# xxlong0/NeuralUDF

Hardware: AMD Instinct MI355X
Metric: ray-samples/sec (train step) (higher is better)
Workload: dtype f32 emulated on the 16-bit matrix pipe, f32 accumulate, f32 state / epilogues / optimizer.  Forward-order sweeps (UDF value, input gradient, colour / NeRF forward): f16x2 (x = hi + 2^-11 lo in fp16, 3 fp16 MFMA products, correction terms in their own accumulator).  Backward sweeps (tangent, adjoint

## Files before the change

### include/nudf.h

```cpp
#ifndef NUDF_H
#define NUDF_H
#include <stdint.h>

#ifdef __cplusplus
extern "C" {
#endif

#define NUDF_ABI_VERSION 111
int nudf_version(void);
#define NUDF_ABI_STRUCTS(X) \
  X(NudfGemmNN) X(NudfGemmTN) X(NudfGemmTNProblem) X(NudfGemmTNGroup) X(NudfComposite) X(NudfCompositeGrad) \
  X(NudfUpsample) X(NudfPixelBlend) X(NudfPixelComposite) X(NudfPatchBlend) X(NudfPatchWarp) X(NudfBlendLoss) \
  X(NudfAdamTensor) X(NudfAdamGroup) X(NudfAdam) X(NudfChainStep) X(NudfChain) X(NudfPackFrag) X(NudfPackLayer) \
  X(NudfPackMulti) X(NudfUnpackLayer) X(NudfUnpackMulti) X(NudfRayBatch) X(NudfMeshUDF) X(NudfMeshUDFSparse) \
  X(NudfIsoSurface) X(NudfIsoSurfaceSparse) X(NudfPointCloud) X(NudfMeshTopo) X(NudfMeshOrient) X(NudfMeshRaster)
int nudf_abi_struct(int i, const char** name);
const char* nudf_last_error(void);

enum {
  NUDF_STATUS_NONFINITE_RENDER = 1,
  NUDF_STATUS_NONFINITE_SAMPLES = 2,
  NUDF_STATUS_NONFINITE_LOSS = 4
};
int nudf_set_status_flag(int32_t* device_word);
// ... 354 lines not shown
  const float* X3;
  int32_t ldx3;
} NudfChainStep;
#define NUDF_CH_BLK_X1 1
#define NUDF_CH_BLK_X2 2
#define NUDF_CH_BLK_C1 4
#define NUDF_CH_BLK_C2 8
#define NUDF_CH_BLK_PE 16
#define NUDF_CH_STATE16 32
#define NUDF_CH_P4_X1 64
#define NUDF_CH_P4_C1 128
typedef struct NudfChain {
  int32_t P, n_steps;
  int32_t init;
  int32_t k0;
  int32_t x_div;
  int32_t tile_rows;
  int32_t lda0, ldg0;
  int32_t pe_L, pe_jvp;
  int32_t init_state16;
  float pe_in_scale;
  float seed_scale, seed_xscale;
  const float* A0;
  float* G0;
  const float* x;
  const float* v;
  const float* seed_sign;
  const float* seed_wrow;
  unsigned long long* dbg;
  float* absmax_out;
  const float* tile_amax_in;
  float* tile_amax_out;
  int32_t tile_scale;
  int32_t reserved0;
  NudfChainStep step[NUDF_CH_MAX_STEPS];
} NudfChain;
#define NUDF_CH_TILE_TQ 66
#define NUDF_CH_TILE_ROWS 128
#if defined(__cplusplus)
static_assert(sizeof(NudfChain) <= 4096, "NudfChain travels by value: the kernel-argument segment holds 4 KB");
#endif
int nudf_mlp_chain(const NudfChain* args, void* stream);
int nudf_mlp_chain_plan(const NudfChain* args, char* name, int capacity, int32_t* out);
int nudf_set_chain_t16(int on);
int nudf_pack_frag(const float* B, int ldb, int K, int N, float* out, void* stream);

#define NUDF_PACK_MAX_LAYERS 16
#define NUDF_PACK_MAX_FRAGS 4
typedef struct NudfPackFrag {
  float* dst;
  int32_t transpose;
  int32_t o0, i0;
  int32_t K, N;
  int32_t dtype;
} NudfPackFrag;
typedef struct NudfPackLayer {
  const float* v; const float* g;
  const int32_t* perm;
  float* W; float* Wt;
  float* inv_norm;
  int32_t out, in, ldw, ldwt;
  int32_t nfrag, row_start;
  NudfPackFrag frag[NUDF_PACK_MAX_FRAGS];
} NudfPackLayer;
typedef struct NudfPackMulti {
  int32_t n_layers, total_rows;
  NudfPackLayer layer[NUDF_PACK_MAX_LAYERS];
// ... 508 lines not shown
```

### neuraludf_amd/_lib.py

```python
from __future__ import annotations

import ctypes as C
import os

import torch

_HERE = os.path.dirname(os.path.abspath(__file__))
LIB_PATH = os.environ.get("NUDF_LIB") or os.path.join(_HERE, "libnudf.so")
ABI_VERSION = 111

c_fp = C.c_void_p
i32 = C.c_int32
f32 = C.c_float


class NudfError(RuntimeError):
    pass


class GemmNN(C.Structure):
    _fields_ = [("A", c_fp), ("lda", i32), ("B", c_fp), ("ldb", i32), ("bias", c_fp),
                ("C1", c_fp), ("ldc1", i32), ("C2", c_fp), ("ldc2", i32), ("C3", c_fp), ("ldc3", i32),
                ("X1", c_fp), ("ldx1", i32), ("X2", c_fp), ("ldx2", i32),
                ("M", i32), ("N", i32), ("K", i32), ("epi", i32), ("iparam", i32), ("scale", f32), ("xscale", f32)]
# ... 101 lines not shown

class AdamGroup(C.Structure):
    _fields_ = [("one_minus_beta1", f32), ("beta2", f32), ("one_minus_beta2", f32), ("eps", f32)]


class Adam(C.Structure):
    _fields_ = [("n_tensors", i32), ("pad_", i32), ("t", AdamTensor * ADAM_MAX_TENSORS),
                ("block_start", i32 * (ADAM_MAX_TENSORS + 1)), ("pad2_", i32), ("group", AdamGroup * ADAM_MAX_GROUPS),
                ("dyn", c_fp)]


CH_MAX_STEPS = 20
CH_STATE16 = 32
CH_P4_X1, CH_P4_C1 = 64, 128
CH = dict(NONE=0, SOFTPLUS=1, MULSP=2, TANGENT=3, BWD=4, UDFHEAD=5, RELU=6, SIGMOIDN=7, MULMASK=8, ADDMASK=9, RELUADD=10,
          SEED=11)
CH_INIT = dict(LOAD=0, POSENC=1, SEED=2)


class ChainStep(C.Structure):
    _fields_ = [("Bp", c_fp), ("bias", c_fp), ("X1", c_fp), ("X2", c_fp), ("C1", c_fp), ("C2", c_fp),
                ("r1_row", c_fp), ("r1_col", c_fp), ("K", i32), ("N", i32), ("epi", i32), ("iparam", i32),
                ("ldx1", i32), ("ldx2", i32), ("ldc1", i32), ("ldc2", i32), ("ldr1", i32), ("prec", i32), ("act_write", i32),
                ("act_col0", i32), ("pe_tail_col", i32), ("ld_pe", i32), ("pe_dst", c_fp), ("pe_tail_scale", f32),
                ("scale", f32), ("xscale", f32), ("layout", i32), ("row_w", c_fp), ("row_sums", c_fp), ("X3", c_fp),
                ("ldx3", i32)]


class Chain(C.Structure):
    _fields_ = [("P", i32), ("n_steps", i32), ("init", i32), ("k0", i32), ("x_div", i32), ("tile_rows", i32), ("lda0", i32),
                ("ldg0", i32), ("pe_L", i32), ("pe_jvp", i32), ("init_state16", i32), ("pe_in_scale", f32), ("seed_scale", f32),
                ("seed_xscale", f32), ("A0", c_fp), ("G0", c_fp), ("x", c_fp), ("v", c_fp), ("seed_sign", c_fp),
                ("seed_wrow", c_fp), ("dbg", c_fp), ("absmax_out", c_fp), ("tile_amax_in", c_fp),
                ("tile_amax_out", c_fp), ("tile_scale", C.c_int32), ("reserved0", C.c_int32), ("step", ChainStep * CH_MAX_STEPS)]


PACK_MAX_LAYERS = 16
PACK_MAX_FRAGS = 4


class PackFrag(C.Structure):
    _fields_ = [("dst", c_fp), ("transpose", i32), ("o0", i32), ("i0", i32), ("K", i32), ("N", i32), ("dtype", i32)]


class PackLayer(C.Structure):
    _fields_ = [("v", c_fp), ("g", c_fp), ("perm", c_fp), ("W", c_fp), ("Wt", c_fp), ("inv_norm", c_fp),
                ("out", i32), ("in_", i32), ("ldw", i32), ("ldwt", i32), ("nfrag", i32), ("row_start", i32),
                ("frag", PackFrag * PACK_MAX_FRAGS)]


class PackMulti(C.Structure):
    _fields_ = [("n_layers", i32), ("total_rows", i32), ("layer", PackLayer * PACK_MAX_LAYERS)]


class UnpackLayer(C.Structure):
    _fields_ = [("dW", c_fp), ("v", c_fp), ("g", c_fp), ("inv_norm", c_fp), ("perm", c_fp), ("dv", c_fp),
                ("dg", c_fp), ("db_in", c_fp), ("db_out", c_fp), ("out", i32), ("in_", i32), ("ldw", i32), ("row_start", i32)]


class UnpackMulti(C.Structure):
    _fields_ = [("n_layers", i32), ("total_rows", i32), ("layer", UnpackLayer * PACK_MAX_LAYERS)]


class MeshUDF(C.Structure):
    _fields_ = [("U", c_fp), ("G", c_fp), ("axes", c_fp), ("cell_case", c_fp), ("cell_ntri", c_fp), ("edge_flag", c_fp),
                ("cells", c_fp), ("face_off", c_fp), ("edge_scan", c_fp), ("faces", c_fp), ("edges", c_fp), ("verts", c_fp),
                ("n_cells", C.c_int64), ("n_edges", C.c_int64), ("n_faces", C.c_int64), ("N", i32), ("mean_thr", f32),
# ... 332 lines not shown
```

### neuraludf_amd/csrc/mlp_chain.hip

```cpp
#include "nudf_common.h"
#include "../../include/nudf.h"

#include "mlp_chain_shared.h"
#include <stdlib.h>
#include <type_traits>

template <int TM>
struct ChainSmem {
  float act[TM * CH_LD];
  float xs[TM * 3];
  float vs[TM * 3];
  float red[8];
};
#define CH_SGN_COL 288
static_assert(CH_SGN_COL < CH_LD, "the head multiplier lives in the tile's row padding");

template <int TM>
struct ChainSmem16 {
  unsigned short act[TM * CH_LD16];
  float xs[TM * 3];
  float vs[TM * 3];
  float red[8];
};

template <int TM, class SM>
__device__ __forceinline__ void ch_write_pe(SM& sm, const NudfChain& p, int m0, int col0, float scale,
                                            float* gdst, int ldg, int gcol0, int zero_to, bool dst16 = false, int tfmt = 0,
                                            float gscale = 1.0f) {
  ch_write_pe_rows<CH_THREADS>(reinterpret_cast<float*>(sm.act), sm.xs, sm.vs, TM, threadIdx.x, p, m0, col0, scale, gdst, ldg,
                               gcol0, zero_to, dst16, false, tfmt, gscale);
}


struct ChPrefetch {
  const float* X1;
  int ldx1;
  unsigned vo[2][2];
};

template <int NRT, int NCT, bool PF>
__device__ __forceinline__ void ch_mma(const float* __restrict__ arow, const f32x4* __restrict__ bptr, size_t bstride,
                                       int G, f32x16 (&acc)[2][2], const ChPrefetch& pf, float (&px1)[2][2][16]) {
  f32x4 a0[NRT], a1[NRT], b0[NCT], b1[NCT];
#pragma unroll
  for (int i = 0; i < NRT; ++i) a0[i] = *reinterpret_cast<const f32x4*>(arow + i * 32 * CH_LD);
#pragma unroll
  for (int j = 0; j < NCT; ++j) b0[j] = bptr[j * 64];
#pragma unroll 1
  for (int g = 0; g < G - 2; g += 2) {
    {
      const f32x4* bq = bptr + (size_t)(g + 1) * bstride;
#pragma unroll
      for (int j = 0; j < NCT; ++j) b1[j] = bq[j * 64];
#pragma unroll
      for (int i = 0; i < NRT; ++i) a1[i] = *reinterpret_cast<const f32x4*>(arow + i * 32 * CH_LD + (g + 1) * 8);
    }
    __builtin_amdgcn_sched_barrier(0);
#pragma unroll
    for (int jj = 0; jj < 4; ++jj)
#pragma unroll
      for (int i = 0; i < NRT; ++i)
#pragma unroll
        for (int j = 0; j < NCT; ++j) acc[i][j] = ch_mfma(a0[i][jj], b0[j][jj], acc[i][j]);
// ... 1016 lines not shown
    for (int e = tid; e < TM * k4; e += CH_THREADS) {
      const int r = e / k4, c4 = e - r * k4;
      int gr = m0 + r;
      if (gr > p.P - 1) gr = p.P - 1;
      const f32x4 val = *reinterpret_cast<const f32x4*>(p.A0 + (size_t)gr * p.lda0 + c4 * 4);
      if constexpr (X3) amax = fmaxf(amax, fmaxf(fmaxf(fabsf(val[0]), fabsf(val[1])), fmaxf(fabsf(val[2]), fabsf(val[3]))));
      if constexpr (T16) {
        uint2 w;
        if (tile_bf) {
          w.x = (unsigned)ch_f2bf(val[0]) | ((unsigned)ch_f2bf(val[1]) << 16);
          w.y = (unsigned)ch_f2bf(val[2]) | ((unsigned)ch_f2bf(val[3]) << 16);
        } else {
          w.x = ch_f2h2(val[0], val[1]);
          w.y = ch_f2h2(val[2], val[3]);
        }
        *reinterpret_cast<uint2*>(sm.act + r * CH_LD16 + c4 * 4) = w;
      } else {
        *reinterpret_cast<f32x4*>(act_f + r * CH_LD + c4 * 4) = val;
      }
    }
    if constexpr (X3) {
      if (tscale) {
        set_sigma(wg_max(fmaxf(amax, other_seeds())));
        for (int e = tid; e < TM * k4; e += CH_THREADS) {
          const int r = e / k4, c4 = e - r * k4;
          f32x4* q = reinterpret_cast<f32x4*>(act_f + r * CH_LD + c4 * 4);
          f32x4 val = *q;
          val[0] *= tsig; val[1] *= tsig; val[2] *= tsig; val[3] *= tsig;
          *q = val;
        }
      }
    }
  } else if (p.init == NUDF_CH_INIT_POSENC) {
    ch_write_pe<TM>(sm, p, m0, 0, 1.0f, p.G0, p.ldg0, 0, p.k0, false, tfmt, tinv);
  } else if (p.init == NUDF_CH_INIT_SEED) {
    const int C = p.k0;
    if ((p.init_state16 & 3) == 3 && p.G0) {
      const uint2* A4 = reinterpret_cast<const uint2*>(p.A0);
      uint2* G4 = reinterpret_cast<uint2*>(p.G0);
      for (int e = tid; e < (TM / 4) * C; e += CH_THREADS) {
        const int q = e / C, c = e - q * C;
        const unsigned gq = (unsigned)(m0 >> 2) + (unsigned)q;
        float hst[4], val[4];
        ch_p4_widen(A4[(size_t)gq * p.lda0 + c], hst);
#pragma unroll
        for (int k = 0; k < 4; ++k) {
          int gr = m0 + 4 * q + k;
          if (gr > p.P - 1) gr = p.P - 1;
          float sd, om;
          ch_sp_derivs(hst[k], p.seed_xscale, sd, om);
          val[k] = p.seed_sign[gr] * p.seed_wrow[c] * p.seed_scale * sd;
          const int r = 4 * q + k;
          if constexpr (T16) sm.act[r * CH_LD16 + c] = tile_bf ? ch_f2bf(val[k]) : ch_f2h(val[k]);
          else act_f[r * CH_LD + c] = val[k];
        }
        uint2 w;
        w.x = (unsigned)ch_f2bf(val[0]) | ((unsigned)ch_f2bf(val[1]) << 16);
        w.y = (unsigned)ch_f2bf(val[2]) | ((unsigned)ch_f2bf(val[3]) << 16);
        G4[(size_t)gq * p.ldg0 + c] = w;
      }
    } else
    for (int e = tid; e < TM * C; e += CH_THREADS) {
      const int r = e / C, c = e - r * C;
      int gr = m0 + r;
      const bool live = gr < p.P;
      if (!live) gr = p.P - 1;
      float s, om;
      const float hst = (p.init_state16 & 1) ? ch_bf2f(reinterpret_cast<const unsigned short*>(p.A0)[ch_p4_off(gr, c, p.lda0)])
                                             : p.A0[(size_t)gr * p.lda0 + c];
      ch_sp_derivs(hst, p.seed_xscale, s, om);
      const float val = p.seed_sign[gr] * p.seed_wrow[c] * p.seed_scale * s;
      if constexpr (T16) sm.act[r * CH_LD16 + c] = tile_bf ? ch_f2bf(val) : ch_f2h(val);
      else act_f[r * CH_LD + c] = val;
      if (p.G0 && live) {
        if (p.init_state16 & 2) reinterpret_cast<unsigned short*>(p.G0)[ch_p4_off(gr, c, p.ldg0)] = ch_f2bf(val);
        else p.G0[(size_t)gr * p.ldg0 + c] = val;
      }
    }
  }
  __syncthreads();

  const unsigned slot = __builtin_amdgcn_s_getreg((3 << 11) | (0 << 6) | 4);
  if (gridDim.x > 256) {
    constexpr unsigned STAGGER16 = 0u, STAGGER32 = 2u;
    const unsigned k = (ANY16 || X3) ? (slot & 1u) * STAGGER16 : ((TM == 64) ? (slot & 1u) * STAGGER32 : slot % 3u);
    for (unsigned d = 0; d < k; ++d) __builtin_amdgcn_s_sleep(127);
  }

  unsigned long long* dbg = p.dbg ? p.dbg + ((size_t)blockIdx.x * 4 + wave) * 64 : nullptr;
  if (dbg && lane == 0) {
    dbg[0] = __builtin_amdgcn_s_getreg((31 << 11) | (0 << 6) | 4);
    dbg[1] = __builtin_amdgcn_s_memtime();
    dbg[62] = wall_clock64();
  }

  for (int si = 0; si < p.n_steps; ++si) {
    const NudfChainStep& st = p.step[si];
    if ((si + slot) & 1u) __builtin_amdgcn_s_setprio(1); else __builtin_amdgcn_s_setprio(0);
    if constexpr (X3) {
      if (st.epi == NUDF_CH_SEED) {
        int t = tid;
        asm volatile("" : "+v"(t));
        const int C = st.N;
        if (t < C) {
          const float wc = st.r1_col[t];
          float* ap = act_f + t;
          float* gp = st.C1 ? st.C1 + (size_t)m0 * st.ldc1 + t : nullptr;
#pragma unroll 4
          for (int r = 0; r < TM; ++r) {
            float s, om;
            ch_sp_derivs(ap[r * CH_LD], st.xscale, s, om);
            const float val = ap[r * CH_LD + CH_SGN_COL - t] * wc * st.scale * s;
            ap[r * CH_LD] = val;
            if (gp) gp[(size_t)r * st.ldc1] = val;
          }
        }
        __syncthreads();
        continue;
      }
    }
    const int G = st.K >> 3;
    const int NT = (st.N + 31) >> 5;
    const f32x4* __restrict__ Bp = reinterpret_cast<const f32x4*>(st.Bp);

    int rt0, ct0, nrt, nct;
    if (WMT == 2) {
      if (NT <= 2) { rt0 = wave >> 1; ct0 = wave & 1; nrt = 1; nct = (ct0 < NT) ? 1 : 0; }
      else if (NT <= 4) { rt0 = wave >> 1; ct0 = 2 * (wave & 1); nrt = 1; nct = min(2, max(0, NT - ct0)); }
      else { rt0 = 0; ct0 = 2 * wave; nrt = 2; nct = min(2, max(0, NT - ct0)); }
    } else {
      rt0 = 0; nrt = 1;
      if (NT <= 4) { ct0 = wave; nct = (ct0 < NT) ? 1 : 0; }
      else { ct0 = 2 * wave; nct = min(2, max(0, NT - ct0)); }
    }

    f32x16 acc[2][2];
// ... 84 lines not shown
        else ch_mma<1, 1, true>(arow, bptr, bstride, G, acc, pf, px1);
      } else {
        if (nrt == 2 && nct == 2) ch_mma<2, 2, false>(arow, bptr, bstride, G, acc, pf, px1);
        else if (nrt == 2) ch_mma<2, 1, false>(arow, bptr, bstride, G, acc, pf, px1);
        else if (nct == 2) ch_mma<1, 2, false>(arow, bptr, bstride, G, acc, pf, px1);
        else ch_mma<1, 1, false>(arow, bptr, bstride, G, acc, pf, px1);
      }
    }
    if (dbg && lane == 0 && si < 14) dbg[2 + 4 * si] = __builtin_amdgcn_s_memtime();
    __syncthreads();
    if (dbg && lane == 0 && si < 14) dbg[3 + 4 * si] = __builtin_amdgcn_s_memtime();

    if (nct > 0) {
      switch (st.epi) {
        case NUDF_CH_SOFTPLUS: ch_epilogue<NUDF_CH_SOFTPLUS, MODE>(p, st, act_f, m0, rt0, ct0, nrt, nct, h, ln, acc, px1, bpre, tile_bf, tsig, tinv); break;
        case NUDF_CH_NONE: { const float em = ch_epilogue<NUDF_CH_NONE, MODE>(p, st, act_f, m0, rt0, ct0, nrt, nct, h, ln, acc, px1, bpre, tile_bf, tsig, tinv); if constexpr (X3) amax = fmaxf(amax, em); } break;
        case NUDF_CH_MULSP: { const float em = ch_epilogue<NUDF_CH_MULSP, MODE>(p, st, act_f, m0, rt0, ct0, nrt, nct, h, ln, acc, px1, bpre, tile_bf, tsig, tinv); if constexpr (X3) amax = fmaxf(amax, em); } break;
        case NUDF_CH_TANGENT:
          if constexpr (MODE != 3) ch_epilogue<NUDF_CH_TANGENT, MODE>(p, st, act_f, m0, rt0, ct0, nrt, nct, h, ln, acc, px1, bpre, tile_bf, tsig, tinv);
          break;
        case NUDF_CH_BWD: { const float em = ch_epilogue<NUDF_CH_BWD, MODE>(p, st, act_f, m0, rt0, ct0, nrt, nct, h, ln, acc, px1, bpre, tile_bf, tsig, tinv); if constexpr (X3) amax = fmaxf(amax, em); } break;
        case NUDF_CH_RELU: ch_epilogue<NUDF_CH_RELU, MODE>(p, st, act_f, m0, rt0, ct0, nrt, nct, h, ln, acc, px1, bpre, tile_bf, tsig, tinv); break;
        case NUDF_CH_SIGMOIDN: ch_epilogue<NUDF_CH_SIGMOIDN, MODE>(p, st, act_f, m0, rt0, ct0, nrt, nct, h, ln, acc, px1, bpre, tile_bf, tsig, tinv); break;
        case NUDF_CH_MULMASK: { const float em = ch_epilogue<NUDF_CH_MULMASK, MODE>(p, st, act_f, m0, rt0, ct0, nrt, nct, h, ln, acc, px1, bpre, tile_bf, tsig, tinv); if constexpr (X3) amax = fmaxf(amax, em); } break;
        case NUDF_CH_ADDMASK: { const float em = ch_epilogue<NUDF_CH_ADDMASK, MODE>(p, st, act_f, m0, rt0, ct0, nrt, nct, h, ln, acc, px1, bpre, tile_bf, tsig, tinv); if constexpr (X3) amax = fmaxf(amax, em); } break;
        case NUDF_CH_RELUADD: ch_epilogue<NUDF_CH_RELUADD, MODE>(p, st, act_f, m0, rt0, ct0, nrt, nct, h, ln, acc, px1, bpre, tile_bf, tsig, tinv); break;
        default: ch_epilogue<NUDF_CH_UDFHEAD, MODE>(p, st, act_f, m0, rt0, ct0, nrt, nct, h, ln, acc, px1, bpre, tile_bf, tsig, tinv); break;
      }
    }
    if (dbg && lane == 0 && si < 14) dbg[4 + 4 * si] = __builtin_amdgcn_s_memtime();
    if (st.pe_tail_col >= 0) {
      __syncthreads();
      const int pe_end = st.pe_tail_col + 3 * (2 * p.pe_L + 1);
      ch_write_pe<TM>(sm, p, m0, st.pe_tail_col, st.pe_tail_scale, st.pe_dst, st.ld_pe, st.pe_tail_col,
                      min((pe_end + 15) & ~15, 288), (st.layout & NUDF_CH_STATE16) != 0, tfmt, tinv);
    }
    __syncthreads();
    if (dbg && lane == 0 && si < 14) dbg[5 + 4 * si] = __builtin_amdgcn_s_memtime();
  }
  if (dbg && lane == 0) dbg[63] = wall_clock64();
  if constexpr (X3) {
    if (p.tile_amax_out) {
      const float m = wg_max(amax);
      if (tid < TM / 32) p.tile_amax_out[(m0 >> 5) + tid] = m;
    }
    if (p.absmax_out) {
#pragma unroll
      for (int off = 32; off > 0; off >>= 1) amax = fmaxf(amax, __shfl_xor(amax, off));
      if (lane == 0 && amax > 0.0f && amax < 3.0e38f) atomicMax(reinterpret_cast<unsigned*>(p.absmax_out), __builtin_bit_cast(unsigned, amax));
    }
  }
}

static const ChainKernel g_shared_kernels[CK_TQ] = {
    CH_KERNEL(32, CH_THREADS, mlp_chain_kernel<32, 2>), CH_KERNEL(32, CH_THREADS, mlp_chain_kernel<32, 1>),
    CH_KERNEL(32, CH_THREADS, mlp_chain_kernel<32, 0>),
    CH_KERNEL(64, CH_THREADS, mlp_chain_kernel<64, 2>), CH_KERNEL(64, CH_THREADS, mlp_chain_kernel<64, 4>),
    CH_KERNEL(64, CH_THREADS, mlp_chain_kernel<64, 3>), CH_KERNEL(64, CH_THREADS, mlp_chain_kernel<64, 1>),
    CH_KERNEL(64, CH_THREADS, mlp_chain_kernel<64, 0>),
};
static const ChainKernel& chain_kernel(int id) { return id < CK_TQ ? g_shared_kernels[id] : nudf_chain_tq_kernel(id); }

struct ChainSettings { int rows_auto, quad, t16, win2; };
static ChainSettings& chain_settings() {
  static ChainSettings s = [] {
    auto env = [](const char* name) { const char* e = getenv(name); return e ? e : ""; };
// ... 106 lines not shown
  if (rows_ok && f.cls >= 0) return f.cls < 2 ? CK_ROWS + f.cls : set.win2 == 3 ? CK_ROWS_2_WIN3 : CK_ROWS_2_WIN2;
  if (f.blocked) return CK_TQ + f.cls;
  if (f.cls >= 0 && !f.roww && !f.fused && (tile == NUDF_CH_TILE_TQ || (tile == 0 && p.P > 256 * 64 && set.quad > 0)) &&
      (tile == NUDF_CH_TILE_TQ || f.cls <= 1 || set.quad >= 2))
    return CK_TQ + f.cls;
  const bool small = tile == 32 || (tile != 64 && p.P <= 256 * 64);
  bool t16 = f.any16 && !f.roww && !small && set.t16;
  bool t16_tangent = false;
  for (int i = 0; i < p.n_steps && t16; ++i) {
    t16 = (p.step[i].prec == 1 || p.step[i].prec == 2) && p.step[i].prec == p.step[0].prec;
    t16_tangent = t16_tangent || p.step[i].epi == NUDF_CH_TANGENT || p.step[i].X3 != nullptr;
  }
  if (small) return f.any3 ? CK_32_M2 : f.any16 ? CK_32_M1 : CK_32_M0;
  return f.any3 ? CK_64_M2 : t16 ? (t16_tangent ? CK_64_M4 : CK_64_M3) : f.any16 ? CK_64_M1 : CK_64_M0;
}

static int chain_plan(const NudfChain& p, int& id) {
  id = -1;
  if (p.P <= 0 || p.n_steps <= 0) return 0;
  ChainFacts f;
  const int err = chain_check(p, f);
  if (!err) id = chain_select(p, f, chain_settings());
  return err;
}

extern "C" int nudf_mlp_chain_plan(const NudfChain* args, char* name, int capacity, int32_t* out) {
  int id;
  const int err = chain_plan(*args, id);
  const ChainKernel* k = id >= 0 ? &chain_kernel(id) : nullptr;
  nudf_report_kernel(name, capacity, out, k ? k->name : nullptr, k ? (args->P + k->points - 1) / k->points : 0, k ? k->threads : 0, 0);
  return err;
}

extern "C" int nudf_mlp_chain(const NudfChain* args, void* stream) {
  int id;
  const int err = chain_plan(*args, id);
  if (err || id < 0) return err;
  const ChainKernel& k = chain_kernel(id);
  k.launch(*args, (args->P + k.points - 1) / k.points, (hipStream_t)stream);
  NUDF_CHECK_LAUNCH("nudf_mlp_chain");
  return 0;
}

__global__ void pack_frag_kernel(const float* __restrict__ B, int ldb, int K, int N, int NT, int total,
                                 float* __restrict__ out) {
  const int idx = blockIdx.x * blockDim.x + threadIdx.x;
  if (idx >= total) return;
  const int j = idx & 3, lane = (idx >> 2) & 63, gt = idx >> 8;
  const int T = gt % NT, g = gt / NT;
  const int k = 8 * g + 4 * (lane >> 5) + j, n = 32 * T + (lane & 31);
  out[idx] = (k < K && n < N) ? B[(size_t)k * ldb + n] : 0.0f;
}

extern "C" int nudf_pack_frag(const float* B, int ldb, int K, int N, float* out, void* stream) {
  if (K <= 0 || N <= 0) return 0;
  const int G = 2 * ((K + 15) / 16), NT = (N + 31) / 32;
  const int total = G * NT * 256;
  hipLaunchKernelGGL(pack_frag_kernel, dim3((total + 255) / 256), dim3(256), 0, (hipStream_t)stream, B, ldb, K, N, NT,
                     total, out);
  NUDF_CHECK_LAUNCH("nudf_pack_frag");
  return 0;
}
```

### neuraludf_amd/csrc/mlp_chain_shared.h

```cpp
#pragma once
#include "nudf_common.h"
#include "../../include/nudf.h"

#define CH_LD 292
#define CH_THREADS 256
#define CH_LD16 296

typedef float f32x8 __attribute__((ext_vector_type(8)));
typedef _Float16 f16x8 __attribute__((ext_vector_type(8)));
typedef __bf16 bf16x8 __attribute__((ext_vector_type(8)));

__device__ __forceinline__ size_t ch_blk_off(int r, int c, int ld) {
  return (size_t)(r >> 5) * 32 * ld + (size_t)(c >> 2) * 128 + (size_t)(r & 31) * 4 + (c & 3);
}

__device__ __forceinline__ size_t ch_p4_off(unsigned row, unsigned col, unsigned ld) {
  return ((size_t)(row >> 2) * ld + col) * 4 + (row & 3);
}
__device__ __forceinline__ float ch_bf2f(unsigned short u) { return __builtin_bit_cast(float, (unsigned)u << 16); }
__device__ __forceinline__ unsigned short ch_f2bf(float x) { return __builtin_bit_cast(unsigned short, (__bf16)x); }

__device__ __forceinline__ f32x16 ch_mfma(float a, float b, f32x16 c) {
  return __builtin_amdgcn_mfma_f32_32x32x2f32(a, b, c, 0, 0, 0);
}
// ... 2 lines not shown
  const float x = 100.0f * xscale * hstored;
  if (x > 20.0f) {
    s = 1.0f;
    om = 0.0f;
  } else {
    const float e = __expf(-x);
    om = e;
    s = (x < 0.01f) ? x * (1.0f - x * (0.5f - x * 0.16666667f)) : 1.0f - e;
  }
}

__device__ __forceinline__ float ch_pe(const float* x3, const float* v3, int c, int L, float in_scale, int jvp) {
  const int blk = c / 3, j = c - blk * 3;
  const float xv = x3[j] * in_scale;
  if (blk == 0) return jvp ? v3[j] * in_scale : xv;
  const int k = (blk - 1) >> 1;
  const float f = (float)(1 << k);
  const float a = xv * f;
  const bool is_sin = ((blk - 1) & 1) == 0;
  if (!jvp) return is_sin ? sinf(a) : cosf(a);
  return (is_sin ? cosf(a) : -sinf(a)) * f * v3[j] * in_scale;
}

__device__ __forceinline__ unsigned ch_f2h2(float a, float b) {
  unsigned r;
  asm("v_cvt_pk_f16_f32 %0, %1, %2" : "=v"(r) : "v"(a), "v"(b));
  return r;
}
__device__ __forceinline__ unsigned short ch_f2h(float x) { return (unsigned short)(ch_f2h2(x, 0.0f) & 0xffffu); }
template <int NTHR>
__device__ __forceinline__ void ch_write_pe_rows(float* act, const float* xs, const float* vs, int rows, int tid,
                                                 const NudfChain& p, int m0, int col0, float scale, float* gdst,
                                                 int ldg, int gcol0, int zero_to, bool dst16 = false,
                                                 bool dstblk = false, int tfmt = 0, float gscale = 1.0f) {
  if (tfmt != 0) {
    unsigned short* a16 = reinterpret_cast<unsigned short*>(act);
    const int L = p.pe_L;
    const int E = 3 * (2 * L + 1);
    for (int it = tid; it < rows * 3 * (L + 1); it += NTHR) {
      const int rj = it / (L + 1), k = it - rj * (L + 1) - 1;
      const int r = rj / 3, j = rj - 3 * r;
      const float xv = xs[rj] * p.pe_in_scale;
      const float tv = vs[rj] * p.pe_in_scale;
      unsigned short* arow = a16 + r * CH_LD16 + col0;
      const bool mirror = gdst && (m0 + r) < p.P;
      const size_t goff = (size_t)(m0 + r) * ldg + gcol0;
      auto put = [&](int c, float val) {
        val *= scale;
        arow[c] = (tfmt == 2) ? ch_f2bf(val) : ch_f2h(val);
        if (mirror) {
          if (dst16) reinterpret_cast<unsigned short*>(gdst)[ch_p4_off(m0 + r, gcol0 + c, ldg)] = ch_f2bf(val);
          else gdst[goff + c] = val;
        }
      };
      if (k < 0) {
        put(j, p.pe_jvp ? tv : xv);
      } else {
        const float f = (float)(1 << k);
        float sn, cs;
        sincosf(xv * f, &sn, &cs);
        put(3 + 6 * k + j, p.pe_jvp ? cs * f * tv : sn);
        put(6 + 6 * k + j, p.pe_jvp ? -sn * f * tv : cs);
      }
    }
    const int npad = zero_to - (col0 + E);
    if (npad > 0)
      for (int e = tid; e < rows * npad; e += NTHR) {
        const int r = e / npad, c = e - r * npad;
        a16[r * CH_LD16 + col0 + E + c] = 0;
      }
    return;
  }
  const int L = p.pe_L;
  const int E = 3 * (2 * L + 1);
  for (int it = tid; it < rows * 3 * (L + 1); it += NTHR) {
    const int rj = it / (L + 1), k = it - rj * (L + 1) - 1;
    const int r = rj / 3, j = rj - 3 * r;
    const float xv = xs[rj] * p.pe_in_scale;
    const float tv = vs[rj] * p.pe_in_scale;
    float* arow = act + r * CH_LD + col0;
    const bool mirror = gdst && (m0 + r) < p.P;
    const size_t goff = (size_t)(m0 + r) * ldg + gcol0;
    auto put = [&](int c, float val) {
      val *= scale;
      arow[c] = val;
      if (mirror) {
        if (dst16) reinterpret_cast<unsigned short*>(gdst)[ch_p4_off(m0 + r, gcol0 + c, ldg)] = ch_f2bf(val);
        else if (dstblk) gdst[ch_blk_off(m0 + r, gcol0 + c, ldg)] = val;
        else gdst[goff + c] = val * gscale;
      }
    };
    if (k < 0) {
      put(j, p.pe_jvp ? tv : xv);
    } else {
      const float f = (float)(1 << k);
      float sn, cs;
      sincosf(xv * f, &sn, &cs);
      put(3 + 6 * k + j, p.pe_jvp ? cs * f * tv : sn);
      put(6 + 6 * k + j, p.pe_jvp ? -sn * f * tv : cs);
    }
  }
  const int npad = zero_to - (col0 + E);
  if (npad > 0)
    for (int e = tid; e < rows * npad; e += NTHR) {
      const int r = e / npad, c = e - r * npad;
      act[r * CH_LD + col0 + E + c] = 0.0f;
    }
}

#define CH_KOFF(r) (((r) & 3) + 8 * ((r) >> 2))

#define CH_USES_X1(e)                                                                                           \
  ((e) == NUDF_CH_MULSP || (e) == NUDF_CH_TANGENT || (e) == NUDF_CH_BWD || (e) == NUDF_CH_MULMASK || (e) == NUDF_CH_ADDMASK)

#define CH_USES_X2(e) ((e) == NUDF_CH_TANGENT || (e) == NUDF_CH_BWD || (e) == NUDF_CH_ADDMASK || (e) == NUDF_CH_RELUADD)

__device__ __forceinline__ void ch_udf_head(int type, float v, float scale, float& out, float& mult) {
  if (type == 1) { out = v * v * scale; mult = 2.0f * v; }
  else if (type == 2) { out = v * scale; mult = 1.0f; }
  else { out = fabsf(v) * scale; mult = (v > 0.0f) ? 1.0f : ((v < 0.0f) ? -1.0f : 0.0f); }
}

struct ChainKernel {
  const char* name;
  int points, threads;
  void (*launch)(const NudfChain& p, int grid, hipStream_t st);
};
template <int THREADS, void (*KERNEL)(NudfChain)>
static void ch_launch(const NudfChain& p, int grid, hipStream_t st) {
  hipLaunchKernelGGL(KERNEL, dim3(grid), dim3(THREADS), 0, st, p);
}
#define CH_KERNEL(points, threads, ...) {#__VA_ARGS__, points, threads, ch_launch<threads, __VA_ARGS__>}
// ... 11 lines not shown
```

### neuraludf_amd/mlp.py

```python
from __future__ import annotations

import math
from typing import List, Optional

import ctypes as C

import torch

from . import _lib
import os

from ._lib import CH, CH_INIT, CH_MAX_STEPS, EPI, Chain, GemmNN, GemmTN, call, ptr


def pad32(n: int) -> int:
    return (n + 31) // 32 * 32


def pad_rows(P: int) -> int:
    return (P + 63) // 64 * 64


def _buf(P, width, dev, zero=None, dtype=torch.float32, blocked=False):
    if blocked:
# ... 162 lines not shown

_PLAIN_TYPES = frozenset((int, float, str, bool, type(None)))
_CHAIN_MEMO = {}
CHAIN_MEMO = os.environ.get("NUDF_CHAIN_MEMO", "1") != "0" and _lib.HOST_FAST
chain_memo_hits = 0


class ChainBuilder:

    def __init__(self, P, init, k0, tile_rows=0, site=None):
        self.P, self.init, self.k0, self.tile_rows = P, init, k0, (tile_rows or CHAIN_TILE)
        self.site = site
        self.rec = []
        self.c = None
        self.n = 0
        self.flops = 0.0
        self.xflops = 0.0
        self.nbytes = 0.0
        self.epis = []
        self.keep = []

    def posenc(self, *a, **kw):
        self.rec.append((0, a, kw))

    def init_store(self, *a, **kw):
        self.rec.append((1, a, kw))

    def init_load(self, *a, **kw):
        self.rec.append((2, a, kw))

    def init_seed(self, *a, **kw):
        self.rec.append((3, a, kw))

    def step(self, *a, **kw):
        self.rec.append((4, a, kw))

    def absmax(self, *a, **kw):
        self.rec.append((5, a, kw))

    def tile_scale(self, *a, **kw):
        self.rec.append((6, a, kw))

    _PARAMS = (("x", "L", "in_scale", "tangent", "x_div"), ("G0",), ("A0", "lda0"),
               ("A0", "lda0", "sign", "wrow", "scale", "xscale"), ("epi", "Bp", "K", "N"), ("t",), ("amax_in", "amax_out"))
    _CHAIN_FIELD = ({"x": "x", "tangent": "v"}, {"G0": "G0"}, {"A0": "A0"}, {"A0": "A0", "sign": "seed_sign", "wrow": "seed_wrow"},
                    None, {"t": "absmax_out"}, {"amax_in": "tile_amax_in", "amax_out": "tile_amax_out"})

    def _signature(self):
        T, PT, plain = torch.Tensor, torch.nn.Parameter, _PLAIN_TYPES
        sig = [self.P, self.init, self.k0, self.tile_rows, PRECISION, FWD_F16X2, BWD_F16X2, HEAD16]
        ptrs = []
        add, addp = sig.append, ptrs.append
        for kind, a, kw in self.rec:
            add(kind)
            for vals in (a, kw.values()):
                for v in vals:
                    tv = type(v)
                    if tv in plain:
                        add(v)
                    elif tv is T or tv is PT or isinstance(v, T):
                        if not (v.is_cuda and v.is_contiguous()):
                            return None, None
                        addp(v.data_ptr())
                        add(v.numel())
                    else:
                        add(v)
            add(tuple(kw))
        return sig, ptrs

    def _fill(self):
        self.c = Chain()
        self.c.P, self.c.init, self.c.k0, self.c.tile_rows = self.P, CH_INIT[self.init], self.k0, self.tile_rows
        self.c.x_div = 1
        fns = (self._do_posenc, self._do_init_store, self._do_init_load, self._do_init_seed, self._do_step, self._do_absmax,
               self._do_tile_scale)
        T = torch.Tensor
        slots = []
        for kind, a, kw in self.rec:
            n0 = self.n
            fns[kind](*a, **kw)
            obj = self.c.step[n0] if kind == 4 else self.c
            names = list(self._PARAMS[kind][:len(a)]) + list(kw)
            vals = list(a) + list(kw.values())
            for nm, v in zip(names, vals):
                if isinstance(v, T):
                    field = nm if kind == 4 else self._CHAIN_FIELD[kind][nm]
                    cur = getattr(obj, field)
                    slots.append((obj, field, cur - v.data_ptr()) if cur is not None else None)
        return slots

    def _p(self, t, off=0):
        if t is None:
            return None
        self.keep.append(t)
        return ptr(t) + t.element_size() * off

    def _do_posenc(self, x, L, in_scale, tangent=None, x_div=1):
        self.c.x, self.c.v = self._p(x), self._p(tangent)
        self.c.pe_L, self.c.pe_jvp, self.c.pe_in_scale = L, (1 if tangent is not None else 0), in_scale
        self.c.x_div = x_div

    def _do_init_store(self, G0):
        if G0 is not None:
            self.c.G0, self.c.ldg0 = self._p(G0), G0.shape[1]
            if _is16(G0) and not _isp4(G0):
                raise _lib.NudfError("a bf16 copy of the initial tile is 4-point packed (mlp.pack16 / _buf)")
# ... 248 lines not shown
            elif kind.startswith("fwd_in:"):
                _, i0, K = kind.split(":")
                f = pack_frag(self.Wt, self.out_pad, int(K), self.out, off=int(i0) * self.out_pad)
            else:
                raise KeyError(kind)
            self._frags[kind] = f
        return f

    @property
    def bias(self):
        return self.lin.bias.detach()

    def new_grad_buffers(self):
        dev = self.W.device
        return torch.zeros(self.out_pad, self.in_pad, device=dev), torch.zeros(self.out, device=dev)


PRECISION = os.environ.get("NUDF_PRECISION", "bf16x3")
_PREC = {"f32": 0, "f16": 1, "bf16": 2, "bf16x3": 3, "f16x2": 4}
FWD_F16X2 = os.environ.get("NUDF_FWD_F16X2", "1")
BWD_F16X2 = os.environ.get("NUDF_BWD_F16X2", "1") != "0"
EX_FLY = os.environ.get("NUDF_EX_FLY", "1") != "0"
TN_F16X2 = True
TN_SPLIT = True
BLOCKED_STATE = True


FUSE_SWEEPS = os.environ.get("NUDF_FUSE_SWEEPS", "1") != "0"


def set_fuse_sweeps(on):
    global FUSE_SWEEPS
    old, FUSE_SWEEPS = FUSE_SWEEPS, bool(on)
    return old


def _shared_split(state=None, mixed16=False):
    return (PRECISION != "fp32" if mixed16 else PRECISION == "bf16x3") and CHAIN_TILE in (0, 32, 64) and not _isblk(state)


def _fuse():
    return FUSE_SWEEPS and _shared_split()


def _tn_prec():
    if PRECISION == "fp32":
        return 0
    return 3 if PRECISION == "bf16x3" else 2


HEAD16 = os.environ.get("NUDF_HEAD16", "1") != "0"


def _head_kind():
    return "fwd_head0@f16" if (PRECISION == "mixed16" and HEAD16) else "fwd_head0"


def _state_blocked(P):
    return PRECISION == "fp32" and USE_CHAIN and CHAIN_TILE in (0, 66) and P > 256 * 64


def _state_dtype():
    return torch.bfloat16 if PRECISION == "mixed16" else torch.float32


def set_precision(name):
# ... 390 lines not shown
        cb.posenc(x, net.multires, float(net.scale))
        if need_grad_state:
            cb.init_store(X[0])
        for l in range(L):
            pl = self.layers[l]
            nxt_skip = (l + 1) in self.skip
            cb.step("SOFTPLUS", pl.frag(_kind("fwd", "fwd")), k8(pl.inp), pl.out, bias=pl.bias,
                    C1=X[l + 1] if need_grad_state else None,
                    scale=self.inv_sqrt2 if nxt_skip else 1.0,
                    pe_tail_col=self._skip_col(l + 1) if nxt_skip else -1, pe_tail_scale=self.inv_sqrt2,
                    pe_dst=X[l + 1] if (need_grad_state and nxt_skip) else None)
        pl = self.layers[L]
        Pp = pad_rows(P)
        udf = torch.empty(Pp, device=dev)
        sign = torch.empty(Pp, device=dev) if need_grad_state else None
        F = pl.out - 1
        feat = None
        if not udf_only:
            ld = max(feat_ld, F)
            if feat_buf is not None and tuple(feat_buf.shape) == (Pp, ld) and ld >= F + 3 and feat_buf.is_contiguous():
                feat = feat_buf
            else:
                feat = torch.empty((Pp, ld), device=dev)
                if ld >= F + 3:
                    call("nudf_copy_cols", ptr(x), 3, 1, ptr(feat) + 4 * F, ld, 3, P, 1.0)
                    _zero_cols(feat, F + 3)
                else:
                    _zero_cols(feat, F)
            cb.step("NONE", pl.frag(_kind("fwd_feat", "fwd")), k8(pl.inp), F, bias=pl.bias, bias_off=1, C1=feat,
                    act_write=0)
        cb.step("UDFHEAD", pl.frag(_head_kind()), k8(pl.inp), 1, bias=pl.bias, C1=sign, C2=udf, ldc1=1, ldc2=1,
                act_write=0, scale=1.0 / float(net.scale), iparam=self.head_type)
        st = dict(udf=udf[:P], sign=(sign[:P] if sign is not None else None),
                  feat=(feat[:P] if feat is not None else None), X=X, P=P)
        if with_grad:
            DA = self._gradient_buffers(P, X, dev)
            n_top = self.layers[L - 1].out
            cb.step("SEED", None, k8(n_top), n_top, r1_col=pl.W, C1=DA[L - 1], scale=1.0 / float(net.scale),
                    xscale=self._xs(L - 1))
            demb0, demb_skip = self._gradient_steps(cb, P, X, DA, dev)
            cb.launch()
            st["g"], st["DA"] = self._gradient_finish(x, P, demb0, demb_skip), DA
            return st
        cb.launch()
        return st

    def _gradient_buffers(self, P, X, dev):
        L = self.L
        return [_buf(P, self.layers[l].out, dev, zero=False, dtype=X[L].dtype, blocked=_isblk(X[L])) for l in range(L)]

    def _gradient_steps(self, cb, P, X, DA, dev):
        Epad = pad32(self.E)
        demb_skip = None
        for l in range(self.L - 1, 0, -1):
            pl = self.layers[l]
            if l in self.skip:
                demb_skip = torch.empty(pad_rows(P), Epad, device=dev)
                cb.step("MULSP", pl.frag(_kind("bwd", "grad")), k8(pl.out), pl.inp, X1=X[l], C1=DA[l - 1], C2=demb_skip,
                        iparam=self.layers[l - 1].out, scale=self.inv_sqrt2, xscale=self._xs(l - 1))
            else:
                cb.step("MULSP", pl.frag(_kind("bwd", "grad")), k8(pl.out), pl.inp, X1=X[l], C1=DA[l - 1],
                        xscale=self._xs(l - 1))
        demb0 = torch.empty(pad_rows(P), Epad, device=dev)
        pl0 = self.layers[0]
        cb.step("NONE", pl0.frag(_kind("bwd", "grad")), k8(pl0.out), pl0.inp, C1=demb0, act_write=0)
        return demb0, demb_skip

# ... 6 lines not shown

    def _gradient_chain(self, x, st):
        P, L, dev = st["P"], self.L, x.device
        X = st["X"]
        net = self.net
        DA = self._gradient_buffers(P, X, dev)
        plL = self.layers[L]
        cb = ChainBuilder(P, "SEED", k8(self.layers[L - 1].out), site=self._site("udf_grad"))
        cb.init_seed(X[L], X[L].shape[1], st["sign"], plL.W, 1.0 / float(net.scale), self._xs(L - 1))
        cb.init_store(DA[L - 1])
        demb0, demb_skip = self._gradient_steps(cb, P, X, DA, dev)
        cb.launch()
        return self._gradient_finish(x, P, demb0, demb_skip), DA

    def _backward_chain(self, x, st, DA, d_udf, d_feat, d_feat_ld, d_g):
        P, L, dev = st["P"], self.L, x.device
        X, sign = st["X"], st["sign"]
        layers = self.layers
        net = self.net
        second = d_g is not None and DA is not None
        R = EX = None
        ex_fly = second and EX_FLY and _shared_split(X[L], mixed16=True)
        tn2 = _shared_split(X[L]) and not _is16(X[L])
        amax = torch.zeros(2, device=dev) if tn2 else None
        bsc = _sweep_dtype("bwd") == "f16x2"
        TA = torch.empty(pad_rows(P) // 32, device=dev) if (bsc and second) else None
        if second:
            sd, blk = X[L].dtype, _isblk(X[L])
            R = ([_buf(P, layers[0].inp, dev, zero=False)] +
                 [_buf(P, pl.inp, dev, zero=False, dtype=sd, blocked=blk) for pl in layers[1:]])
            EX = None if ex_fly else [_buf(P, layers[l].out, dev, zero=False, dtype=sd, blocked=blk) for l in range(L)]
            cb = ChainBuilder(P, "POSENC", k8(self.E), site=self._site("udf_tangent"))
            cb.posenc(x, net.multires, float(net.scale), tangent=d_g.contiguous())
            cb.init_store(R[0])
            if tn2:
                cb.absmax(amax[1:2])
            if bsc:
                cb.tile_scale(amax_out=TA)
            for l in range(L):
                pl = layers[l]
                nxt_skip = (l + 1) in self.skip
                if ex_fly:
                    cb.step("MULSP", pl.frag(_kind("fwd", "bwd")), k8(pl.inp), pl.out, X1=X[l + 1], C1=R[l + 1],
                            scale=self.inv_sqrt2 if nxt_skip else 1.0, xscale=self._xs(l),
                            pe_tail_col=self._skip_col(l + 1) if nxt_skip else -1, pe_tail_scale=self.inv_sqrt2,
                            pe_dst=R[l + 1] if nxt_skip else None)
                else:
                    cb.step("TANGENT", pl.frag(_kind("fwd", "bwd")), k8(pl.inp), pl.out, X1=X[l + 1], X2=DA[l], C1=R[l + 1],
                            C2=EX[l],
                            scale=self.inv_sqrt2 if nxt_skip else 1.0, xscale=self._xs(l),
                            pe_tail_col=self._skip_col(l + 1) if nxt_skip else -1, pe_tail_scale=self.inv_sqrt2,
                            pe_dst=R[l + 1] if nxt_skip else None)
            cb.launch()
        inv_scale = 1.0 / float(net.scale)
        plL = layers[L]
        F = plL.out - 1
        head4 = torch.empty(pad_rows(P), 4, device=dev)
        sg4 = torch.empty(pad_rows(P), 4, device=dev) if second else None
        if d_udf is not None:
            call("nudf_col0_seed4", ptr(sign), ptr(d_udf.reshape(-1).contiguous()), float(inv_scale), P, pad_rows(P),
                 ptr(head4), ptr(sg4))
        else:
            head4.zero_()
            if second:
                call("nudf_col0_seed4", ptr(sign), None, float(inv_scale), P, pad_rows(P), ptr(sg4), None)
        ABAR = [_buf(P, layers[l].out, dev, zero=False, dtype=X[L].dtype, blocked=_isblk(X[L])) for l in range(L)]
# ... 585 lines not shown
```

Measured before the change: 19.77 million.

## Compute positional encoding once per chain and reuse sin/cos from forward activations

Adds a pe_once mode to the MLP chain kernel. The positional-encoding terms are stashed in the tile's row padding so skip-layer tails reuse them rather than recomputing sincos, and the tangent sweep reads sin/cos from the stored forward input X[0] instead of calling sincosf. It also adds a vectorized f32x4 path for the SEED epilogue. The stash is only enabled when a host-side check confirms no step writes into the padding columns, which adds eligibility logic and the risk of clobbered stash data.

```diff
diff --git a/include/nudf.h b/include/nudf.h
--- a/include/nudf.h
+++ b/include/nudf.h
@@ -410,7 +410,7 @@
   const float* tile_amax_in;
   float* tile_amax_out;
   int32_t tile_scale;
-  int32_t reserved0;
+  int32_t pe_once;
   NudfChainStep step[NUDF_CH_MAX_STEPS];
 } NudfChain;
 #define NUDF_CH_TILE_TQ 66
diff --git a/neuraludf_amd/_lib.py b/neuraludf_amd/_lib.py
--- a/neuraludf_amd/_lib.py
+++ b/neuraludf_amd/_lib.py
@@ -157,7 +157,7 @@
                 ("ldg0", i32), ("pe_L", i32), ("pe_jvp", i32), ("init_state16", i32), ("pe_in_scale", f32), ("seed_scale", f32),
                 ("seed_xscale", f32), ("A0", c_fp), ("G0", c_fp), ("x", c_fp), ("v", c_fp), ("seed_sign", c_fp),
                 ("seed_wrow", c_fp), ("dbg", c_fp), ("absmax_out", c_fp), ("tile_amax_in", c_fp),
-                ("tile_amax_out", c_fp), ("tile_scale", C.c_int32), ("reserved0", C.c_int32), ("step", ChainStep * CH_MAX_STEPS)]
+                ("tile_amax_out", c_fp), ("tile_scale", C.c_int32), ("pe_once", C.c_int32), ("step", ChainStep * CH_MAX_STEPS)]
 
 
 PACK_MAX_LAYERS = 16
diff --git a/neuraludf_amd/csrc/mlp_chain.hip b/neuraludf_amd/csrc/mlp_chain.hip
--- a/neuraludf_amd/csrc/mlp_chain.hip
+++ b/neuraludf_amd/csrc/mlp_chain.hip
@@ -26,9 +26,34 @@
 template <int TM, class SM>
 __device__ __forceinline__ void ch_write_pe(SM& sm, const NudfChain& p, int m0, int col0, float scale,
                                             float* gdst, int ldg, int gcol0, int zero_to, bool dst16 = false, int tfmt = 0,
-                                            float gscale = 1.0f) {
+                                            float gscale = 1.0f, float* stash = nullptr, const float* pesrc = nullptr,
+                                            int ldsrc = 0) {
   ch_write_pe_rows<CH_THREADS>(reinterpret_cast<float*>(sm.act), sm.xs, sm.vs, TM, threadIdx.x, p, m0, col0, scale, gdst, ldg,
-                               gcol0, zero_to, dst16, false, tfmt, gscale);
+                               gcol0, zero_to, dst16, false, tfmt, gscale, stash, pesrc, ldsrc);
+}
+
+#define CH_PE_STASH_COL 256
+template <int NTHR, int ROWS>
+__device__ __forceinline__ void ch_pe_from_stash(float* act, const float* xs, const float* vs, int tid, const NudfChain& p,
+                                                 int m0, int col0, float scale, float* gdst, int ldg, int zero_to,
+                                                 float gscale) {
+  constexpr int TPR = NTHR / ROWS;
+  const int r = tid / TPR;
+  const int E = 3 * (2 * p.pe_L + 1);
+  float* arow = act + r * CH_LD;
+  const float* idn = (p.pe_jvp ? vs : xs) + r * 3;
+  const bool mirror = gdst && (m0 + r) < p.P;
+  const size_t goff = (size_t)(m0 + r) * ldg + col0;
+  const int n = zero_to - col0;
+  for (int c = tid % TPR; c < n; c += TPR) {
+    float val = 0.0f;
+    if (c < E) {
+      val = (c < 3) ? idn[c] * p.pe_in_scale : arow[CH_PE_STASH_COL + c - 3];
+      val *= scale;
+      if (mirror) gdst[goff + c] = val * gscale;
+    }
+    arow[col0 + c] = val;
+  }
 }
 
 
@@ -1111,7 +1136,13 @@
       }
     }
   } else if (p.init == NUDF_CH_INIT_POSENC) {
-    ch_write_pe<TM>(sm, p, m0, 0, 1.0f, p.G0, p.ldg0, 0, p.k0, false, tfmt, tinv);
+    float* stash = nullptr;
+    const float* pesrc = nullptr;
+    if constexpr (X3) {
+      stash = (p.pe_once & 1) ? act_f + CH_PE_STASH_COL : nullptr;
+      pesrc = (p.pe_once & 4) ? p.A0 : nullptr;
+    }
+    ch_write_pe<TM>(sm, p, m0, 0, 1.0f, p.G0, p.ldg0, 0, p.k0, false, tfmt, tinv, stash, pesrc, p.lda0);
   } else if (p.init == NUDF_CH_INIT_SEED) {
     const int C = p.k0;
     if ((p.init_state16 & 3) == 3 && p.G0) {
@@ -1166,7 +1197,7 @@
     for (unsigned d = 0; d < k; ++d) __builtin_amdgcn_s_sleep(127);
   }
 
-  unsigned long long* dbg = p.dbg ? p.dbg + ((size_t)blockIdx.x * 4 + wave) * 64 : nullptr;
+  unsigned long long* dbg = p.dbg ? p.dbg + ((size_t)blockIdx.x * 4 + __builtin_amdgcn_readfirstlane(wave)) * 64 : nullptr;
   if (dbg && lane == 0) {
     dbg[0] = __builtin_amdgcn_s_getreg((31 << 11) | (0 << 6) | 4);
     dbg[1] = __builtin_amdgcn_s_memtime();
@@ -1181,6 +1212,30 @@
         int t = tid;
         asm volatile("" : "+v"(t));
         const int C = st.N;
+        if ((p.pe_once & 2) && !(C & 3) && !(st.ldc1 & 3) && !(((uintptr_t)st.C1 | (uintptr_t)st.r1_col) & 15)) {
+          const int q = (t & 63) * 4;
+          if (q < C) {
+            const f32x4 wc = *reinterpret_cast<const f32x4*>(st.r1_col + q);
+            float* ap = act_f + (t >> 6) * CH_LD;
+            float* gp = st.C1 ? st.C1 + (size_t)(m0 + (t >> 6)) * st.ldc1 + q : nullptr;
+#pragma unroll 1
+            for (int r = 0; r < TM / 4; ++r) {
+              const f32x4 hv = *reinterpret_cast<const f32x4*>(ap + q);
+              const float sg = ap[CH_SGN_COL];
+              f32x4 val;
+#pragma unroll
+              for (int k = 0; k < 4; ++k) {
+                float s, om;
+                ch_sp_derivs(hv[k], st.xscale, s, om);
+                val[k] = sg * wc[k] * st.scale * s;
+              }
+              *reinterpret_cast<f32x4*>(ap + q) = val;
+              if (gp) *reinterpret_cast<f32x4*>(gp) = val;
+              ap += 4 * CH_LD;
+              if (gp) gp += (size_t)4 * st.ldc1;
+            }
+          }
+        } else
         if (t < C) {
           const float wc = st.r1_col[t];
           float* ap = act_f + t;
@@ -1331,6 +1386,14 @@
     if (st.pe_tail_col >= 0) {
       __syncthreads();
       const int pe_end = st.pe_tail_col + 3 * (2 * p.pe_L + 1);
+      bool stashed = false;
+      if constexpr (X3) stashed = (p.pe_once & 1) != 0;
+      int t = tid;
+      asm volatile("" : "+v"(t));
+      if (stashed)
+        ch_pe_from_stash<CH_THREADS, TM>(act_f, sm.xs, sm.vs, t, p, m0, st.pe_tail_col, st.pe_tail_scale, st.pe_dst, st.ld_pe,
+                                         min((pe_end + 15) & ~15, 288), tinv);
+      else
       ch_write_pe<TM>(sm, p, m0, st.pe_tail_col, st.pe_tail_scale, st.pe_dst, st.ld_pe, st.pe_tail_col,
                       min((pe_end + 15) & ~15, 288), (st.layout & NUDF_CH_STATE16) != 0, tfmt, tinv);
     }
@@ -1503,11 +1566,34 @@
   return err;
 }
 
+static bool chain_pe_stash_ok(const NudfChain& p) {
+  if (p.init != NUDF_CH_INIT_POSENC || !p.x || p.pe_L < 1 || 6 * p.pe_L > CH_LD - CH_PE_STASH_COL || p.k0 > CH_PE_STASH_COL)
+    return false;
+  int last = -1;
+  for (int i = 0; i < p.n_steps; ++i)
+    if (p.step[i].pe_tail_col >= 0) last = i;
+  const int E = 3 * (2 * p.pe_L + 1);
+  for (int i = 0; i <= last; ++i) {
+    const NudfChainStep& s = p.step[i];
+    if (s.epi != NUDF_CH_NONE && s.epi != NUDF_CH_SOFTPLUS && s.epi != NUDF_CH_MULSP && s.epi != NUDF_CH_TANGENT) return false;
+    if (s.K > CH_PE_STASH_COL || (s.layout & NUDF_CH_STATE16)) return false;
+    if (s.act_write && s.act_col0 + ((s.N + 31) & ~31) > CH_PE_STASH_COL) return false;
+    if (s.pe_tail_col >= 0 && ((s.pe_tail_col + E + 15) & ~15) > CH_PE_STASH_COL) return false;
+  }
+  return last >= 0;
+}
+
 extern "C" int nudf_mlp_chain(const NudfChain* args, void* stream) {
   int id;
   const int err = chain_plan(*args, id);
   if (err || id < 0) return err;
   const ChainKernel& k = chain_kernel(id);
+  if (args->pe_once) {
+    NudfChain q = *args;
+    const bool src = q.init == NUDF_CH_INIT_POSENC && q.pe_jvp && q.A0 && q.x && q.pe_L > 0 && q.lda0 >= 3 * (2 * q.pe_L + 1);
+    q.pe_once = (id == CK_32_M2 || id == CK_64_M2) ? (2 | (chain_pe_stash_ok(q) ? 1 : 0) | (src ? 4 : 0)) : 0;
+    k.launch(q, (q.P + k.points - 1) / k.points, (hipStream_t)stream);
+  } else
   k.launch(*args, (args->P + k.points - 1) / k.points, (hipStream_t)stream);
   NUDF_CHECK_LAUNCH("nudf_mlp_chain");
   return 0;
diff --git a/neuraludf_amd/csrc/mlp_chain_shared.h b/neuraludf_amd/csrc/mlp_chain_shared.h
--- a/neuraludf_amd/csrc/mlp_chain_shared.h
+++ b/neuraludf_amd/csrc/mlp_chain_shared.h
@@ -58,7 +58,8 @@
 __device__ __forceinline__ void ch_write_pe_rows(float* act, const float* xs, const float* vs, int rows, int tid,
                                                  const NudfChain& p, int m0, int col0, float scale, float* gdst,
                                                  int ldg, int gcol0, int zero_to, bool dst16 = false,
-                                                 bool dstblk = false, int tfmt = 0, float gscale = 1.0f) {
+                                                 bool dstblk = false, int tfmt = 0, float gscale = 1.0f,
+                                                 float* stash = nullptr, const float* pesrc = nullptr, int ldsrc = 0) {
   if (tfmt != 0) {
     unsigned short* a16 = reinterpret_cast<unsigned short*>(act);
     const int L = p.pe_L;
@@ -121,9 +122,19 @@
     } else {
       const float f = (float)(1 << k);
       float sn, cs;
+      if (pesrc) {
+        const size_t so = (size_t)min(m0 + r, p.P - 1) * ldsrc + 6 * k + j;
+        sn = pesrc[so + 3];
+        cs = pesrc[so + 6];
+      } else
       sincosf(xv * f, &sn, &cs);
-      put(3 + 6 * k + j, p.pe_jvp ? cs * f * tv : sn);
-      put(6 + 6 * k + j, p.pe_jvp ? -sn * f * tv : cs);
+      const float e0 = p.pe_jvp ? cs * f * tv : sn, e1 = p.pe_jvp ? -sn * f * tv : cs;
+      if (stash) {
+        stash[r * CH_LD + 6 * k + j] = e0;
+        stash[r * CH_LD + 6 * k + j + 3] = e1;
+      }
+      put(3 + 6 * k + j, e0);
+      put(6 + 6 * k + j, e1);
     }
   }
   const int npad = zero_to - (col0 + E);
diff --git a/neuraludf_amd/mlp.py b/neuraludf_amd/mlp.py
--- a/neuraludf_amd/mlp.py
+++ b/neuraludf_amd/mlp.py
@@ -218,6 +218,9 @@
     def init_seed(self, *a, **kw):
         self.rec.append((3, a, kw))
 
+    def pe_source(self, *a, **kw):
+        self.rec.append((2, a, kw))
+
     def step(self, *a, **kw):
         self.rec.append((4, a, kw))
 
@@ -234,7 +237,7 @@
 
     def _signature(self):
         T, PT, plain = torch.Tensor, torch.nn.Parameter, _PLAIN_TYPES
-        sig = [self.P, self.init, self.k0, self.tile_rows, PRECISION, FWD_F16X2, BWD_F16X2, HEAD16]
+        sig = [self.P, self.init, self.k0, self.tile_rows, PRECISION, FWD_F16X2, BWD_F16X2, HEAD16, PE_ONCE]
         ptrs = []
         add, addp = sig.append, ptrs.append
         for kind, a, kw in self.rec:
@@ -258,6 +261,7 @@
         self.c = Chain()
         self.c.P, self.c.init, self.c.k0, self.c.tile_rows = self.P, CH_INIT[self.init], self.k0, self.tile_rows
         self.c.x_div = 1
+        self.c.pe_once = 1 if PE_ONCE else 0
         fns = (self._do_posenc, self._do_init_store, self._do_init_load, self._do_init_seed, self._do_step, self._do_absmax,
                self._do_tile_scale)
         T = torch.Tensor
@@ -572,6 +576,15 @@
 def set_fuse_sweeps(on):
     global FUSE_SWEEPS
     old, FUSE_SWEEPS = FUSE_SWEEPS, bool(on)
+    return old
+
+
+PE_ONCE = os.environ.get("NUDF_PE_ONCE", "1") != "0"
+
+
+def set_pe_once(on):
+    global PE_ONCE
+    old, PE_ONCE = PE_ONCE, bool(on)
     return old
 
 
@@ -1028,7 +1041,7 @@
         cb.step("UDFHEAD", pl.frag(_head_kind()), k8(pl.inp), 1, bias=pl.bias, C1=sign, C2=udf, ldc1=1, ldc2=1,
                 act_write=0, scale=1.0 / float(net.scale), iparam=self.head_type)
         st = dict(udf=udf[:P], sign=(sign[:P] if sign is not None else None),
-                  feat=(feat[:P] if feat is not None else None), X=X, P=P)
+                  feat=(feat[:P] if feat is not None else None), X=X, P=P, x0_chain=True)
         if with_grad:
             DA = self._gradient_buffers(P, X, dev)
             n_top = self.layers[L - 1].out
@@ -1101,6 +1114,8 @@
             EX = None if ex_fly else [_buf(P, layers[l].out, dev, zero=False, dtype=sd, blocked=blk) for l in range(L)]
             cb = ChainBuilder(P, "POSENC", k8(self.E), site=self._site("udf_tangent"))
             cb.posenc(x, net.multires, float(net.scale), tangent=d_g.contiguous())
+            if PE_ONCE and st.get("x0_chain") and _shared_split(X[L]) and X[0].dtype == torch.float32 and not _isblk(X[0]):
+                cb.pe_source(X[0], X[0].shape[1])
             cb.init_store(R[0])
             if tn2:
                 cb.absmax(amax[1:2])
```

Measured after the change: 19.71 million (median of 3 runs). About the same (-0.3%).
